# matthewhoung/inference-arena

Measured on AMD Instinct MI355X. Metric: req/sec (whole node) + P50/P99 e2e latency, YOLOv5n→MobileNetV2 at 1/2/4/8 GPU, higher is better.
Workload: dtype fp32

## Files before the change

### csrc/kernels/conv_f32.hip

```cpp
#include <algorithm>
#include <cstdlib>
#include <stdexcept>
#include <string>

#include "common.h"
#include "launch.h"
#include "letterbox.h"

namespace arena {

__device__ __forceinline__ float4 load_f4_or_zero(const float* p, const float* safe, bool ok) {
  const float4 v = *(const float4*)(ok ? p : safe);
  return ok ? v : make_float4(0.f, 0.f, 0.f, 0.f);
}

__device__ __forceinline__ float f4_get(const float4& v, int s) {
  return s == 0 ? v.x : s == 1 ? v.y : s == 2 ? v.z : v.w;
}

__device__ __forceinline__ int xcd_remap(int bx, int nx) {
  const int q = nx / 8, r = nx % 8, x = bx % 8, y = bx / 8;
  return (x < r ? x * (q + 1) : r * (q + 1) + (x - r) * q) + y;
}

// ... 1351 lines not shown
}

static bool f32_stream(const ConvParams& p, hipStream_t s) {
  if (p.Cin % 4 != 0 || p.Kpad > 192 || p.Kpad % 16 != 0 || p.Kpad < p.KH * p.KW * p.Cin || p.xs % 4 != 0)
    return false;
  const int ncf = p.Cout_pad / 16;
  const int nf = ncf <= 5 ? ncf : ncf % 4 == 0 ? 4 : ncf % 3 == 0 ? 3 : ncf % 5 == 0 ? 5 : ncf % 2 == 0 ? 2 : 1;
  switch (nf) {
    case 1: return launch_stream_exact_k<1>(p, s);
    case 2: return launch_stream_exact_k<2>(p, s);
    case 3: return launch_stream_exact_k<3>(p, s);
    case 4: return launch_stream_exact_k<4>(p, s);
    case 5: return launch_stream_exact_k<5>(p, s);
    default: return false;
  }
}

static bool x3_stream(const ConvParams& p, hipStream_t s, int nf_force) {
  if (p.Cin % 8 != 0 || p.Kpad > 192 || p.Kpad < p.KH * p.KW * p.Cin || p.xs % 4 != 0) return false;
  const int ncf = p.Cout_pad / 16;
  const int nf = nf_force ? nf_force
                          : ncf <= 5 ? ncf : ncf % 4 == 0 ? 4 : ncf % 3 == 0 ? 3 : ncf % 5 == 0 ? 5 : ncf % 2 == 0 ? 2 : 1;
  switch (nf) {
    case 1: return launch_stream_k<1>(p, s);
    case 2: return launch_stream_k<2>(p, s);
    case 3: return launch_stream_k<3>(p, s);
    case 4: return launch_stream_k<4>(p, s);
    case 5: return launch_stream_k<5>(p, s);
    default: return false;
  }
}

void conv2d_f32(const ConvParams& p, hipStream_t s) {
  if (p.Cin % 4 != 0 || p.xs % 4 != 0 || p.Kpad % 16 != 0 || p.Cout_pad % 16 != 0 || p.Cout % 4 != 0 ||
      p.Cout > p.Cout_pad || p.ys % 4 != 0)
    throw std::runtime_error("conv2d_f32: unsupported geometry (Cin/xs/ys %4, Kpad %16, Cout_pad %16, Cout %4)");
  if (p.Cin < 16) throw std::runtime_error("conv2d_f32: Cin must be >= 16");
  if (p.Kpad < p.KH * p.KW * p.Cin) throw std::runtime_error("conv2d_f32: Kpad < KH*KW*Cin");
  if (p.pw_w != nullptr) {
    if (p.impl >= kF32X3HRPw && p.impl < kF32X3HRPw + kF32X3HRPwVariants) {
      if (!conv_x3hr_pw(p, s, p.impl - kF32X3HRPw))
        throw std::runtime_error("conv2d_f32: a fused pointwise epilogue needs an x3hr-pw variant that fits the conv");
      return;
    }
    const int v = p.impl >= kF32X3HGPw && p.impl < kF32X3HGPw + kF32X3HGPwVariants ? p.impl - kF32X3HGPw
                  : p.impl >= kF32X3HGPwSmall && p.impl < kF32X3HGPwSmall + kF32X3HGPwSmallVariants
                      ? kF32X3HGPwVariants + p.impl - kF32X3HGPwSmall
                  : p.impl == 0 ? (p.Cout_pad <= 64 ? 0 : 2)
                                : -1;
    if (v < 0 || !conv_x3hg_pw(p, s, v))
      throw std::runtime_error("conv2d_f32: a fused pointwise epilogue needs an x3hg-pw variant that fits the conv");
    return;
  }
  if (p.res != nullptr && p.rs % 4 != 0) throw std::runtime_error("conv2d_f32: residual stride % 4");
  if (p.y2 != nullptr && p.y2s % 4 != 0) throw std::runtime_error("conv2d_f32: upsampled stride % 4");
  const long M = (long)p.B * p.Ho * p.Wo;
  if (M <= 0) return;
  if (M > 0x7fffffffL || (long)p.B * p.H * p.W * p.xs > 0x7fffffffL) throw std::runtime_error("conv2d_f32: too large");
  const int ncf = p.Cout_pad / 16;
  if (p.lb_meta != nullptr) {
    if (p.lb_pool == nullptr || !x3_h16(p, s))
      throw std::runtime_error("conv2d_f32: a letterbox-source conv must be a 3x3 s1 pad-1 conv over 16 channels");
    return;
  }
  if (p.impl >= 10) {
    if (p.impl >= kF32X3G && p.impl < kF32X3G + kF32X3GVariants) {
      if (!conv_x3g(p, s, p.impl - kF32X3G))
        throw std::runtime_error("conv2d_f32: not an x3g-eligible conv (needs pre-split weights)");
      return;
    }
    if (p.impl >= kF32X3GSK && p.impl < kF32X3GSK + kF32X3GSKVariants) {
      if (!conv_x3g_sk(p, s, p.impl - kF32X3GSK))
        throw std::runtime_error("conv2d_f32: not a split-K x3g-eligible conv (pre-split weights, workspace)");
      return;
    }
    if (p.impl >= kF32X3HG && p.impl < kF32X3HG + kF32X3HGVariants) {
      if (!conv_x3hg(p, s, p.impl - kF32X3HG))
        throw std::runtime_error("conv2d_f32: not an x3hg-eligible conv (3x3 s1 with pre-split weights)");
      return;
    }
    if (p.impl >= kF32X3HR && p.impl < kF32X3HR + kF32X3HRVariants) {
      if (!conv_x3hr(p, s, p.impl - kF32X3HR))
        throw std::runtime_error("conv2d_f32: not an x3hr-eligible conv (3x3 s1 with pre-split weights)");
      return;
    }
    if (p.impl == kF32X3H16) {
      if (!x3_h16(p, s)) throw std::runtime_error("conv2d_f32: not an x3-h16-eligible conv (3x3 s1 over 16 channels)");
      return;
    }
    if (p.impl == kF32Fc) {
      if (!conv_fc_f32(p, s)) throw std::runtime_error("conv2d_f32: not an FC-eligible conv (1x1 map, Kpad 1280)");
      return;
    }
    if (p.impl == kF32StreamExact) {
      if (!f32_stream(p, s)) throw std::runtime_error("conv2d_f32: not a stream-eligible conv (Cin % 4, Kpad <= 192)");
      return;
    }
    if (p.impl == kF32Stream || p.impl == kF32StreamN2) {
      if (!x3_stream(p, s, p.impl == kF32StreamN2 ? 2 : 0))
        throw std::runtime_error("conv2d_f32: not a stream-eligible conv (Cin % 8, Kpad <= 192)");
      return;
    }
    if (p.impl == kF32X3Halo || p.impl == kF32X3HaloN3 || p.impl == kF32X3HaloN2 || p.impl == kF32X3Halo16 ||
        p.impl == kF32X3Halo16N3) {
      const int nf = (p.impl == kF32X3HaloN3 || p.impl == kF32X3Halo16N3) ? 3 : p.impl == kF32X3HaloN2 ? 2 : 0;
      const int th = (p.impl == kF32X3Halo16 || p.impl == kF32X3Halo16N3) ? 16 : 8;
      if (!x3_halo(p, s, nf, th)) throw std::runtime_error("conv2d_f32: not an x3-halo-eligible conv");
      return;
    }
    if (p.impl == kF32Halo) {
      if (!halo_f32(p, s, true)) throw std::runtime_error("conv2d_f32: not a halo-eligible conv");
      return;
    }
    if (p.impl >= kF32X3) {
      if (p.impl >= kF32X3 + kF32X3Variants || !launch_x3_variant(p, s, M, p.impl - kF32X3))
        throw std::runtime_error("conv2d_f32: unknown x3 variant");
      return;
    }
    if (p.impl >= 10 + kF32Variants || !launch_lds_variant(p, s, M, p.impl - 10)) throw std::runtime_error("conv2d_f32: unknown variant");
    return;
  }
  if (p.impl == 0 && conv_fc_f32(p, s)) return;
  const int impl = p.impl == 1 ? 1 : p.impl >= 2 ? 2 : f32_conv_family();
  if (impl == 2 && halo_f32(p, s)) return;
  if (impl == 2) {
    if (ncf == 1)
      launch_lds_m<1, 4, 1>(p, s, M);
    else if (ncf == 2)
      launch_lds_m<2, 4, 1>(p, s, M);
    else if (ncf == 3 || ncf == 9)
      launch_lds_m<3, 4, 1>(p, s, M);
    else if (ncf == 5)
      launch_lds_m<5, 4, 1>(p, s, M);
    else if (ncf == 6)
      launch_lds_m<3, 2, 2>(p, s, M);
    else
      launch_lds_m<2, 2, 2>(p, s, M);
    return;
  }
  if (ncf % 4 == 0 || ncf > 12)
    launch_f32_wc<4>(p, s, M);
  else if (ncf % 3 == 0)
    launch_f32_wc<3>(p, s, M);
  else if (ncf % 2 == 0)
    launch_f32_wc<2>(p, s, M);
  else if (ncf == 5)
    launch_f32_wc<5>(p, s, M);
  else
    launch_f32_wc<1>(p, s, M);
}

template <int R, int S, int CX>
__global__ __launch_bounds__(256) void dwconv_f32_kernel(const DwParams p) {
  const int B = live_batch(p.B, p.bdev);
  const int cg = p.C >> 2;
  const int strips = (p.Ho + R - 1) / R;
  const int colb = (p.Wo + CX - 1) / CX;
  const int total = B * strips * colb * cg;
  const int tid = blockIdx.x * blockDim.x + threadIdx.x;
  if (tid >= total) return;
  const int g = tid % cg;
  int t = tid / cg;
  const int ox0 = (t % colb) * CX;
  t /= colb;
  const int st = t % strips;
  const int b = t / strips;
// ... 151 lines not shown
```

### csrc/kernels/detect.hip

```cpp
#include <string>
#include <stdexcept>
#include "common.h"
#include "launch.h"

namespace arena {

constexpr int SPPF_MAX_PIX = 1024;

__global__ __launch_bounds__(256) void sppf_kernel(const SppfParams p) {
  extern __shared__ __align__(16) uint4 sp[];
  const int B = live_batch(p.B, p.bdev);
  const int groups = p.C >> 4;
  const int b = blockIdx.x / groups;
  if (b >= B) return;
  const int c0 = (blockIdx.x - b * groups) * 16;
  const int H = p.H, W = p.W, HW = H * W;
  uint4* in = sp;
  uint4* h5 = sp + 2 * HW;
  uint4* h9 = sp + 4 * HW;
  uint4* h13 = sp + 6 * HW;
  bf16* buf = (bf16*)p.buf + (size_t)b * HW * p.xs;
  constexpr int kIt = (SPPF_MAX_PIX * 2 + 255) / 256;
  uint4 tmp[kIt];
#pragma unroll
// ... 171 lines not shown
  int P = 2;
  while (P < n) P <<= 1;
  unsigned long long* keys = (unsigned long long*)smem;
  unsigned char* removed = smem + sizeof(unsigned long long) * P;
  const Candidate* cand = p.cand + (size_t)b * p.cand_cap;

  for (int i = tid; i < P; i += NMS_THREADS) {
    unsigned long long k = ~0ull;
    if (i < n) {
      const Candidate c = cand[i];
      const unsigned bits = __float_as_uint(c.score);
      unsigned diff = bits <= 0x3F800000u ? 0x3F800000u - bits : 0u;
      diff = diff < (1u << 29) ? diff : (1u << 29) - 1u;
      k = ((unsigned long long)(unsigned)(c.cls & 127) << 57) | ((unsigned long long)diff << 28) |
          ((unsigned long long)(unsigned)(c.anchor & 0x3FFF) << 14) | (unsigned long long)i;
      removed[i] = 0;
    }
    keys[i] = k;
  }
  __syncthreads();
  for (int k = 2; k <= P; k <<= 1) {
    for (int j = k >> 1; j > 0; j >>= 1) {
      for (int i = tid; i < P; i += NMS_THREADS) {
        const int ixj = i ^ j;
        if (ixj > i) {
          const unsigned long long a = keys[i], c = keys[ixj];
          const bool up = (i & k) == 0;
          if ((a > c) == up) { keys[i] = c; keys[ixj] = a; }
        }
      }
      __syncthreads();
    }
  }

  const ImageMeta m = p.meta[b];
  const float scale = m.scale;
  int kept = 0;
  for (int i = 0; i < n; ++i) {
    if (removed[i]) continue;
    const unsigned long long ki = keys[i];
    const int ci = (int)(ki >> 57);
    const Candidate bi = cand[ki & 0x3FFF];
    if (tid == 0 && kept < p.max_det) {
      Detection d;
      d.x1 = fminf(fmaxf((bi.x1 - (float)m.pad_w) / scale, 0.f), (float)m.w);
      d.y1 = fminf(fmaxf((bi.y1 - (float)m.pad_h) / scale, 0.f), (float)m.h);
      d.x2 = fminf(fmaxf((bi.x2 - (float)m.pad_w) / scale, 0.f), (float)m.w);
      d.y2 = fminf(fmaxf((bi.y2 - (float)m.pad_h) / scale, 0.f), (float)m.h);
      d.conf = bi.score;
      d.cls = bi.cls;
      d.pad_[0] = d.pad_[1] = 0.f;
      p.det[(size_t)b * p.max_det + kept] = d;
    }
    ++kept;
    const float area_i = (bi.x2 - bi.x1) * (bi.y2 - bi.y1);
    for (int j = i + 1 + tid; j < n; j += NMS_THREADS) {
      const unsigned long long kj = keys[j];
      if ((int)(kj >> 57) != ci) break;
      if (removed[j]) continue;
      const Candidate bj = cand[kj & 0x3FFF];
      const float xx1 = fmaxf(bi.x1, bj.x1), yy1 = fmaxf(bi.y1, bj.y1);
      const float xx2 = fminf(bi.x2, bj.x2), yy2 = fminf(bi.y2, bj.y2);
      const float inter = fmaxf(0.f, xx2 - xx1) * fmaxf(0.f, yy2 - yy1);
      const float area_j = (bj.x2 - bj.x1) * (bj.y2 - bj.y1);
      const float iou = inter / (area_i + area_j - inter + 1e-6f);
      if (iou > p.iou_thr) removed[j] = 1;
    }
    __syncthreads();
  }
  if (tid == 0) p.det_count[b] = kept;
}

void prepare_kernels() {
  static bool done = false;
  if (done) return;
  ARENA_HIP_CHECK(hipFuncSetAttribute((const void*)nms_kernel, hipFuncAttributeMaxDynamicSharedMemorySize,
                                      160 * 1024));
  ir_prepare();
  head_pool_f32_prepare();
  x3_halo_prepare();
  x3g_prepare();
  c3_x3_prepare();
  x3hg_prepare();
  stem_s2_f32_prepare();
  ARENA_HIP_CHECK(hipFuncSetAttribute((const void*)sppf_kernel, hipFuncAttributeMaxDynamicSharedMemorySize,
                                      160 * 1024));
  done = true;
}

void nms(const NmsParams& p, hipStream_t s) {
  if (p.cand_cap > 16384) throw std::runtime_error("nms: cand_cap > 16384");
  int P = 2;
  while (P < p.cand_cap) P <<= 1;
  const size_t lds = (size_t)P * 9;
  if (lds > 160 * 1024) throw std::runtime_error("nms: LDS budget exceeded");
  if (p.B <= 0) return;
  hipLaunchKernelGGL(nms_kernel, dim3(p.B), dim3(NMS_THREADS), lds, s, p);
}

__global__ __launch_bounds__(256) void crop_plan_kernel(const CropPlanParams p) {
  __shared__ int offs[1024 + 1];
  const int n_img = live_batch(p.B, p.ctrl ? &p.ctrl->n_images : nullptr);
  const int tid = threadIdx.x;
  if (p.whole) {
    for (int b = tid; b < n_img; b += blockDim.x) {
      const ImageMeta m = p.meta[b];
      Detection d;
      d.x1 = 0.f; d.y1 = 0.f; d.x2 = (float)m.w; d.y2 = (float)m.h;
      d.conf = 1.f; d.cls = -1; d.pad_[0] = d.pad_[1] = 0.f;
      p.det[(size_t)b * p.max_det] = d;
      p.det_count[b] = 1;
      CropRef r;
      r.img = b; r.x1 = 0; r.y1 = 0; r.x2 = m.w; r.y2 = m.h; r.det = 0; r.pad_[0] = r.pad_[1] = 0;
      p.crops[b] = r;
    }
    if (tid == 0) {
      Ctrl* c = p.ctrl;
      c->total_crops = n_img;
      int rem = n_img - c->crop_base;
      rem = rem < 0 ? 0 : rem;
      c->n_crops = rem < p.crop_cap ? rem : p.crop_cap;
    }
    return;
  }
  for (int b = tid; b < n_img; b += blockDim.x) {
    const int k = p.det_count[b];
    offs[b + 1] = k < p.max_det ? k : p.max_det;
  }
  if (tid == 0) offs[0] = 0;
  __syncthreads();
  if (tid < 64) {
    int carry = 0;
    for (int base = 0; base < n_img; base += 64) {
      const int i = base + tid;
      int v = i < n_img ? offs[i + 1] : 0;
#pragma unroll
      for (int o = 1; o < 64; o <<= 1) {
        const int u = __shfl_up(v, o, 64);
        if (tid >= o) v += u;
      }
      if (i < n_img) offs[i + 1] = v + carry;
      carry += __shfl(v, 63, 64);
    }
    if (tid == 0) {
      Ctrl* c = p.ctrl;
      c->total_crops = carry;
      int rem = carry - c->crop_base;
      rem = rem < 0 ? 0 : rem;
      c->n_crops = rem < p.crop_cap ? rem : p.crop_cap;
    }
  }
  __syncthreads();
  const int total = offs[n_img];
  for (int i = tid; i < total; i += blockDim.x) {
    int lo = 0, hi = n_img - 1;
    while (lo < hi) {
      const int mid = (lo + hi + 1) >> 1;
      if (offs[mid] <= i) lo = mid;
      else hi = mid - 1;
    }
    const int b = lo, d = i - offs[lo];
    const ImageMeta m = p.meta[b];
    const Detection det = p.det[(size_t)b * p.max_det + d];
    CropRef r;
    r.img = b;
    r.x1 = max(0, (int)det.x1);
// ... 78 lines not shown
```

### csrc/kernels/launch.h

```cpp
#pragma once
#include <hip/hip_runtime.h>
#include <stdint.h>
#include <stdexcept>
#include <string>

namespace arena {

struct ImageMeta;
struct CropRef;
struct Ctrl;
struct ConvParams {
  const void* x;
  int B, H, W;
  int xs;
  int Cin;
  const void* w;
  int Kpad;
  const float* bias;
  void* y;
  int Ho, Wo, ys;
  int Cout;
  int Cout_pad;
  int KH, KW, stride, pad_t, pad_l;
  const void* res;
  int rs;
  void* y2;
  int y2s;
  int act;
  int f32out;
  const int* bdev;
  int impl;
  const void* pw_w;
  const float* pw_bias;
  void* pw_y;
  int pw_ys, pw_cout, pw_kpad, pw_act;
  const uint8_t* lb_pool;
  const ImageMeta* lb_meta;
  const void* w3;
  float* sk_ws;
  int64_t sk_ws_bytes;
  int sk_splits;
};
void conv2d(const ConvParams& p, hipStream_t s);
void conv_igemm(const ConvParams& p, hipStream_t s);
bool conv_pw(const ConvParams& p, hipStream_t s);
void set_conv_pw(bool v);
bool conv3x3_v3(const ConvParams& p, hipStream_t s);
bool conv_fc(const ConvParams& p, hipStream_t s);
void set_conv_v3(bool v);
void set_conv_impl(int v);
int get_conv_impl();

constexpr int kF32Variants = 16;
constexpr int kF32X3 = 40;
constexpr int kF32X3Variants = 12;
constexpr int kF32Halo = 100;
constexpr int kF32X3Halo = 101;
constexpr int kF32X3HaloN3 = 102;
constexpr int kF32X3HaloN2 = 103;
constexpr int kF32Stream = 104;
constexpr int kF32StreamN2 = 105;
constexpr int kF32Fc = 106;
constexpr int kF32StreamExact = 107;
constexpr int kF32X3Halo16 = 108;
constexpr int kF32X3Halo16N3 = 109;
constexpr int kF32X3H16 = 110;
constexpr int kF32X3G = 111;
constexpr int kF32X3GVariants = 20;
void x3_halo_prepare();
bool x3g_supported(const ConvParams& p);
bool conv_x3g(const ConvParams& p, hipStream_t s, int v);
constexpr int kF32X3GSK = 171;
constexpr int kF32X3GSKVariants = 9;
bool conv_x3g_sk(const ConvParams& p, hipStream_t s, int v);
void x3g_prepare();
constexpr int kF32X3HG = 131;
constexpr int kF32X3HGVariants = 14;
bool x3hg_supported(const ConvParams& p);
bool conv_x3hg(const ConvParams& p, hipStream_t s, int v);
void x3hg_prepare();
constexpr int kF32X3HGPw = 145;
constexpr int kF32X3HGPwVariants = 6;
constexpr int kF32X3HGPwSmall = 181;
constexpr int kF32X3HGPwSmallVariants = 2;
bool conv_x3hg_pw(const ConvParams& p, hipStream_t s, int v);
constexpr int kF32X3HR = 151;
constexpr int kF32X3HRVariants = 10;
constexpr int kF32X3HRPw = 161;
constexpr int kF32X3HRPwVariants = 6;
bool conv_x3hr(const ConvParams& p, hipStream_t s, int v);
bool conv_x3hr_pw(const ConvParams& p, hipStream_t s, int v);
bool conv_fc_f32(const ConvParams& p, hipStream_t s);
void conv2d_f32(const ConvParams& p, hipStream_t s);

struct DwParams {
  const void* x;
  int B, H, W, xs, C;
  const void* w;
  const float* bias;
  void* y;
  int Ho, Wo, ys, stride, act;
  const int* bdev;
};
void dwconv3x3(const DwParams& p, hipStream_t s);
void dwconv3x3_f32(const DwParams& p, hipStream_t s);

struct IrParams {
  const void* x;
  int x_cs, H, W;
  int inp, inp_pad;
  int hid_pad;
  int oup, oup_pad;
  int stride, expand, res;
  const void* we;
  const float* be;
  const void* wd;
  const float* bd;
  const void* wp;
  const float* bp;
  void* y;
  int y_cs, Ho, Wo;
  int B;
  const int* bdev;
  int x3w;
  int x_parts, y_parts;
  int stem;
  const uint8_t* st_pool;
  const ImageMeta* st_meta;
  const CropRef* st_crops;
  const Ctrl* st_ctrl;
  int st_S;
  float st_mean[3], st_inv_std[3];
  const float* st_w;
  const float* st_b;
};
void ir_block(const IrParams& p, hipStream_t s);
void ir_block_f32(const IrParams& p, hipStream_t s);
bool ir_block_f32_supported(int stride, int inp_pad, int hid_pad, int oup_pad, int expand);
bool ir_block_crop_f32(const IrParams& p, hipStream_t s);
bool ir_block_crop_f32_supported(int H, int stride, int inp_pad, int hid_pad, int oup_pad, int expand);
bool ir_tile_x3(const IrParams& p, hipStream_t s);
bool ir_tile_x3_supported(int stride, int inp_pad, int hid_pad, int oup_pad, int expand);
void ir_tile_x3_prepare();
bool ir_stem_x3(const IrParams& p, hipStream_t s);
void ir_prepare();
void set_ir_t14(bool v);
void set_ir_crop(bool v);
void set_ir_crop_split(int v);
void set_ir_wave(bool v);
void set_irx_slices_big(int n);
void set_irx_parts(int n);

struct C3Params {
  const void* x;
  int xs;
  int B, H, W;
  const int* bdev;
  int C1, CH, NB, res;
  const void* w12;
  const float* b12;
  const void* wb1[2];
  const float* bb1[2];
  const void* wb2[2];
  const float* bb2[2];
  const void* w3;
  const float* b3;
  void* y;
  int ys;
};
bool c3_fused_supported(int C1, int CH, int NB, bool res, int H, int W);
bool c3_x3_supported(int C1, int CH, int NB, bool res, int H, int W);
void c3_x3(const C3Params& p, hipStream_t s);
// ... 221 lines not shown
```

### csrc/runtime/executor.cpp

```cpp
#include "executor.h"
#include "peer.h"

#include <pthread.h>
#include <sys/prctl.h>

#include <algorithm>
#include <chrono>
#include <cmath>
#include <cstdio>
#include <cstdlib>
#include <cstring>
#include <thread>
#include <stdexcept>
#include <string>

#include "../kernels/common.h"
#include "../kernels/jpeg_desc.h"
#include "jpeg_decode.h"
#include "trace.h"

namespace arena {

namespace {
float bits_to_float(int64_t v) {
// ... 219 lines not shown

std::vector<uint8_t> Executor::weights_host() {
  std::vector<uint8_t> out(weights_bytes_);
  if (d_weights_ == nullptr || weights_bytes_ == 0) return out;
  ARENA_HIP_CHECK(hipSetDevice(cfg_.device));
  sync_slots();
  ARENA_HIP_CHECK(hipMemcpy(out.data(), d_weights_, weights_bytes_, hipMemcpyDeviceToHost));
  return out;
}

void Executor::set_program(const int64_t* ops, int n_ops, const int64_t* cls_ops, int n_cls_ops) {
  prog_.resize(n_ops);
  for (int i = 0; i < n_ops; ++i) std::memcpy(prog_[i].data(), ops + (size_t)i * kOpFields, sizeof(OpRecord));
  cls_prog_.resize(n_cls_ops);
  for (int i = 0; i < n_cls_ops; ++i)
    std::memcpy(cls_prog_[i].data(), cls_ops + (size_t)i * kOpFields, sizeof(OpRecord));
  has_topk_ = has_det_ = has_raw_ = has_stamps_ = false;
  for (const auto& r : prog_) {
    has_topk_ |= r[0] == OP_TOPK;
    has_stamps_ |= r[0] == OP_STAMP;
    has_det_ |= r[0] == OP_NMS || r[0] == OP_CROPPLAN;
    for (int f = 1; f < kOpFields; ++f) has_raw_ |= r[f] == BUF_RAWOUT && (r[0] == OP_YOLORAW || r[0] == OP_CONV);
  }
  if (has_raw_ && cfg_.raw_out_bytes <= 0) throw std::runtime_error("program exports raw outputs: raw_out_bytes = 0");
}

int Executor::crop_cap_for(int B) const { return std::max(cfg_.min_crop_cap, B * cfg_.crop_cap_per_image); }

std::vector<int> Executor::buckets() const {
  std::vector<int> r;
  for (auto& kv : buckets_) r.push_back(kv.first);
  return r;
}

uintptr_t Executor::arena_ptr(int B) const {
  auto it = buckets_.find(B);
  return it == buckets_.end() ? 0 : (uintptr_t)it->second.d_arena[0];
}

void Executor::read_arena(int B, int64_t offset, void* dst, size_t bytes) {
  auto it = buckets_.find(B);
  if (it == buckets_.end()) throw std::runtime_error("read_arena: unknown bucket");
  if (offset < 0 || offset + (int64_t)bytes > it->second.info.arena_bytes)
    throw std::runtime_error("read_arena: range outside the arena");
  ARENA_HIP_CHECK(hipSetDevice(cfg_.device));
  sync_slots();
  ARENA_HIP_CHECK(hipMemcpy(dst, it->second.d_arena[it->second.last_slot] + offset, bytes, hipMemcpyDeviceToHost));
}

void Executor::add_bucket(int B, const int64_t* offsets, int n_buffers, int64_t arena_bytes,
                          const std::vector<int>* impl) {
  if (B <= 0 || B > max_B_) throw std::runtime_error("add_bucket: B outside (0, max_batch]");
  if (prog_.empty()) throw std::runtime_error("add_bucket: set_program first");
  if (d_weights_ == nullptr) throw std::runtime_error("add_bucket: set_weights first");
  ARENA_HIP_CHECK(hipSetDevice(cfg_.device));
  Bucket& bk = buckets_[B];
  bk.info.B = B;
  bk.info.crop_cap = crop_cap_for(B);
  bk.info.offsets.assign(offsets, offsets + n_buffers);
  bk.info.arena_bytes = arena_bytes;
  sync_slots();
  free_arenas(bk);
  const size_t abytes = (size_t)std::max<int64_t>(arena_bytes, 256);
  for (int s = 0; s < n_slots_; ++s) {
    ARENA_HIP_CHECK(hipMalloc(&bk.d_arena[s], abytes));
    ARENA_HIP_CHECK(hipMemset(bk.d_arena[s], 0, abytes));
  }
  bk.impl.assign(prog_.size(), 0);
  if (impl != nullptr) {
    if (impl->size() != prog_.size()) throw std::runtime_error("add_bucket: tuning table does not match the program");
    for (size_t i = 0; i < prog_.size(); ++i) {
      const int v = (*impl)[i];
      const bool f32 = prog_[i][kDtypeField] == 1;
      const bool ok = f32 ? (v >= 0 && v <= 2) || (v >= 10 && v < 10 + kF32Variants) ||
                                (v >= kF32X3 && v < kF32X3 + kF32X3Variants) || v == kF32Halo || v == kF32X3Halo ||
                                v == kF32X3HaloN3 || v == kF32X3HaloN2 || v == kF32Stream || v == kF32StreamN2 ||
                                v == kF32Fc || v == kF32StreamExact || v == kF32X3Halo16 || v == kF32X3Halo16N3 ||
                                v == kF32X3H16 || (v >= kF32X3G && v < kF32X3G + kF32X3GVariants) ||
                                (v >= kF32X3HG && v < kF32X3HG + kF32X3HGVariants) ||
                                (v >= kF32X3HGPw && v < kF32X3HGPw + kF32X3HGPwVariants) ||
                                (v >= kF32X3HGPwSmall && v < kF32X3HGPwSmall + kF32X3HGPwSmallVariants) ||
                                (v >= kF32X3HR && v < kF32X3HR + kF32X3HRVariants) ||
                                (v >= kF32X3HRPw && v < kF32X3HRPw + kF32X3HRPwVariants) ||
                                (v >= kF32X3GSK && v < kF32X3GSK + kF32X3GSKVariants)
                          : v >= 0 && v <= 3;
      if (!ok || (v != 0 && prog_[i][0] != OP_CONV)) throw std::runtime_error("add_bucket: bad tuning entry");
      bk.impl[i] = (int16_t)v;
    }
  } else if (autotune_) {
    autotune(bk);
  }
  for (int s = 0; s < n_slots_; ++s) capture(bk, s);
  if (debug_sync_ || std::getenv("ARENA_DEBUG_ALLOC")) {
    fprintf(stderr, "[arena alloc] bucket %d arena %p..%p (%lld B)\n", B, (void*)bk.d_arena[0],
            (void*)(bk.d_arena[0] + arena_bytes), (long long)arena_bytes);
    for (int s = 0; s < n_slots_; ++s)
      fprintf(stderr, "[arena alloc] slot %d in %p..%p out %p..%p\n", s, (void*)slots_[s].d_in,
              (void*)(slots_[s].d_in + in_bytes_total()), (void*)slots_[s].d_out,
              (void*)(slots_[s].d_out + out_bytes_total()));
    fprintf(stderr, "[arena alloc] weights %p..%p\n", (void*)d_weights_, (void*)(d_weights_ + weights_bytes_));
  }
}

void Executor::autotune(Bucket& bk) {
  Slot& sl = slots_[0];
  Ctrl c{};
  c.n_images = bk.info.B;
  c.n_crops = bk.info.crop_cap;
  ARENA_HIP_CHECK(hipStreamSynchronize(compute_));
  ARENA_HIP_CHECK(hipMemcpy(sl.d_in, &c, sizeof(Ctrl), hipMemcpyHostToDevice));
  hipEvent_t e0, e1;
  ARENA_HIP_CHECK(hipEventCreate(&e0));
  ARENA_HIP_CHECK(hipEventCreate(&e1));
  static const int kF32Candidates[] = {0,      12,     13,     14,     17,     19,     20,         21,
                                       23,     24,     kF32Halo, kF32X3, kF32X3 + 1, kF32X3 + 4, kF32X3 + 5,
                                       kF32X3 + 6, kF32X3 + 7, kF32X3 + 8, kF32X3Halo, kF32X3HaloN3,
                                       kF32X3HaloN2, kF32Stream, kF32StreamN2, kF32Fc, kF32StreamExact,
                                       kF32X3Halo16, kF32X3Halo16N3, kF32X3H16,
                                       kF32X3G + 5, kF32X3G + 6, kF32X3G + 7, kF32X3G + 9, kF32X3G + 15,
                                       kF32X3G + 16, kF32X3G + 17, kF32X3G + 19,
                                       kF32X3HG + 0, kF32X3HG + 1, kF32X3HG + 2, kF32X3HG + 4, kF32X3HG + 6,
                                       kF32X3HG + 7, kF32X3HG + 8, kF32X3HG + 9, kF32X3HG + 10,
                                       kF32X3HGPw + 0, kF32X3HGPw + 1, kF32X3HGPw + 2, kF32X3HGPw + 3,
                                       kF32X3HGPw + 4, kF32X3HGPw + 5, kF32X3HGPwSmall + 0, kF32X3HGPwSmall + 1,
                                       kF32X3HR + 0, kF32X3HR + 1, kF32X3HR + 2, kF32X3HR + 3, kF32X3HR + 4,
                                       kF32X3HR + 5, kF32X3HR + 6, kF32X3HR + 7, kF32X3HR + 8, kF32X3HR + 9,
                                       kF32X3HRPw + 0, kF32X3HRPw + 1, kF32X3HRPw + 2, kF32X3HRPw + 3,
                                       kF32X3HRPw + 4, kF32X3HRPw + 5,
                                       kF32X3GSK + 0, kF32X3GSK + 1, kF32X3GSK + 2, kF32X3GSK + 3, kF32X3GSK + 4,
                                       kF32X3GSK + 5, kF32X3GSK + 6, kF32X3GSK + 7, kF32X3GSK + 8};
  static const int kBf16Candidates[] = {1, 2, 3};
  for (size_t i = 0; i < prog_.size(); ++i) {
    if (prog_[i][0] != OP_CONV) continue;
    const bool f32 = prog_[i][kDtypeField] == 1;
    if (prog_[i][1] == BUF_POOL) {
      bk.impl[i] = kF32X3H16;
      continue;
    }
    if (!f32 && prog_[i][34] > 0) {
      bk.impl[i] = 2;
      continue;
    }
    const int reps = f32 ? 5 : 3;
    std::vector<OpRecord> one(1, prog_[i]);
    float best = 1e30f;
    int best_impl = -1;
    const int* cand = f32 ? kF32Candidates : kBf16Candidates;
    const int n_cand = f32 ? (int)(sizeof(kF32Candidates) / sizeof(int)) : 3;
    for (int ci = 0; ci < n_cand; ++ci) {
      const int impl = cand[ci];
      try {
        enqueue_program(one, bk, sl, compute_, (int)i, impl);
      } catch (const std::runtime_error&) {
        continue;
      }
      ARENA_HIP_CHECK(hipEventRecord(e0, compute_));
      for (int k = 0; k < reps; ++k) enqueue_program(one, bk, sl, compute_, (int)i, impl);
      ARENA_HIP_CHECK(hipEventRecord(e1, compute_));
      ARENA_HIP_CHECK(hipEventSynchronize(e1));
      float ms = 0.f;
      ARENA_HIP_CHECK(hipEventElapsedTime(&ms, e0, e1));
      if (best_impl < 0 || ms < best * 0.97f) {
        best = ms;
        best_impl = impl;
      }
    }
    bk.impl[i] = (int16_t)std::max(best_impl, 0);
    if (autotune_ > 1)
      fprintf(stderr, "[arena autotune] B=%d op %zu -> impl %d (%.1f us)\n", bk.info.B, i, best_impl,
              best * 1e3f / reps);
  }
  ARENA_HIP_CHECK(hipEventDestroy(e0));
  ARENA_HIP_CHECK(hipEventDestroy(e1));
  ARENA_HIP_CHECK(hipMemset(bk.d_arena[0], 0, std::max<int64_t>(bk.info.arena_bytes, 256)));
}

static int lanes_max_batch() {
  static const int v = [] {
    const char* e = std::getenv("ARENA_LANES_MAX_BATCH");
    return e != nullptr ? std::atoi(e) : 2;
  }();
  return v;
}

bool Executor::lanes_for(const Bucket& bk) const {
  if (bk.info.B > lanes_max_batch()) return false;
  for (const OpRecord& r : prog_)
    if (r[kLaneField] >= 1 && r[kLaneField] <= kMaxLanes) return true;
  return false;
}

int64_t Executor::sk_lane_bytes() {
  static const int64_t v = [] {
    const char* e = std::getenv("ARENA_SPLITK_WS_MB");
    return (int64_t)std::max(1, e != nullptr ? std::atoi(e) : 16) << 20;
  }();
  return v;
}

void Executor::destroy_graphs(Bucket& bk, int s) {
  if (bk.graph[s]) hipGraphExecDestroy(bk.graph[s]);
  bk.graph[s] = nullptr;
  for (hipGraphExec_t g : bk.parts[s])
    if (g) hipGraphExecDestroy(g);
  bk.parts[s].clear();
  for (auto& sg : bk.segs[s])
    if (sg.g) hipGraphExecDestroy(sg.g);
  bk.segs[s].clear();
}

void Executor::capture(Bucket& bk, int s) {
// ... 1094 lines not shown
```

Before: 10310.

## Add register-prefetched halo 3x3 conv kernel family to fp32 autotune candidates

Adds a new 3x3 stride-1 fp32 conv kernel (x3hp) that stages an input halo tile and weight slices in LDS as bf16x3 splits and uses six MFMA products to emulate fp32 accuracy. Global loads for the next stage are issued into registers before the MFMA work of the current stage, so memory latency can overlap compute. Nine tile and stage variants are registered with the dispatcher and added to the autotune candidate list. The effect depends on the autotuner choosing these variants over existing ones; it adds compile time and LDS pressure per variant.

```diff
diff --git a/csrc/kernels/conv_f32.hip b/csrc/kernels/conv_f32.hip
--- a/csrc/kernels/conv_f32.hip
+++ b/csrc/kernels/conv_f32.hip
@@ -1457,6 +1457,11 @@
     if (p.impl >= kF32X3HR && p.impl < kF32X3HR + kF32X3HRVariants) {
       if (!conv_x3hr(p, s, p.impl - kF32X3HR))
         throw std::runtime_error("conv2d_f32: not an x3hr-eligible conv (3x3 s1 with pre-split weights)");
+      return;
+    }
+    if (p.impl >= kF32X3HP && p.impl < kF32X3HP + kF32X3HPVariants) {
+      if (!conv_x3hp(p, s, p.impl - kF32X3HP))
+        throw std::runtime_error("conv2d_f32: not an x3hp-eligible conv (3x3 s1 with pre-split weights)");
       return;
     }
     if (p.impl == kF32X3H16) {
diff --git a/csrc/kernels/detect.hip b/csrc/kernels/detect.hip
--- a/csrc/kernels/detect.hip
+++ b/csrc/kernels/detect.hip
@@ -277,6 +277,7 @@
   x3g_prepare();
   c3_x3_prepare();
   x3hg_prepare();
+  x3hp_prepare();
   stem_s2_f32_prepare();
   ARENA_HIP_CHECK(hipFuncSetAttribute((const void*)sppf_kernel, hipFuncAttributeMaxDynamicSharedMemorySize,
                                       160 * 1024));
diff --git a/csrc/kernels/halo_x3p.hip b/csrc/kernels/halo_x3p.hip
--- /dev/null
+++ b/csrc/kernels/halo_x3p.hip
@@ -0,0 +1,259 @@
+#include <stdexcept>
+#include <string>
+
+#include "common.h"
+#include "launch.h"
+
+namespace arena {
+
+namespace {
+
+typedef unsigned u32x4 __attribute__((ext_vector_type(4)));
+
+constexpr int HP_TW = 16, HP_HC = HP_TW + 2;
+constexpr int HP_XP = 3 * 32 + 16;
+__host__ __device__ constexpr int hp_wp(int TS) { return TS * 96 + 16; }
+__host__ __device__ constexpr int hp_lds_bytes(int NF, int TH, int TS) {
+  return ((TH + 2) * HP_HC * HP_XP + NF * 16 * hp_wp(TS)) * 2;
+}
+
+__device__ __forceinline__ int hp_xcd_remap(int bx, int nx) {
+  const int q = nx / 8, r = nx % 8, x = bx % 8, y = bx / 8;
+  return (x < r ? x * (q + 1) : r * (q + 1) + (x - r) * q) + y;
+}
+
+}
+
+template <int NF, int TH, int TS>
+__global__ __launch_bounds__(TH * 32) void conv_x3hp_kernel(const ConvParams p) {
+  static_assert(TS == 1 || TS == 3, "a weight stage is one tap or one kernel row");
+  constexpr int NT = TH * 32, NW = TH / 2;
+  constexpr int HR = TH + 2, HPIX = HR * HP_HC;
+  constexpr int XI = (HPIX * 8 + NT - 1) / NT;
+  constexpr int BN = NF * 16, MF = 2;
+  constexpr int WP = hp_wp(TS);
+  constexpr int WPC = TS * BN * 12;
+  constexpr int WI = (WPC + NT - 1) / NT;
+  constexpr int SPC = 9 / TS;
+  extern __shared__ __attribute__((aligned(16))) bf16 hp_lds[];
+  bf16* sX = hp_lds;
+  bf16* sW = hp_lds + HPIX * HP_XP;
+
+  const int tid = threadIdx.x, lane = tid & 63, wave = tid >> 6;
+  const int col = lane & 15, kq = lane >> 4;
+  const int tiles_x = (p.Wo + HP_TW - 1) / HP_TW, tiles_y = (p.Ho + TH - 1) / TH;
+  const int tiles = tiles_x * tiles_y;
+  const int bx = hp_xcd_remap(blockIdx.x, gridDim.x);
+  const int b = bx / tiles;
+  if (b >= live_batch(p.B, p.bdev)) return;
+  const int t = bx - b * tiles;
+  const int ty = t / tiles_x, tx = t - ty * tiles_x;
+  const int oy0 = ty * TH, ox0 = tx * HP_TW;
+  const int iy0 = oy0 - p.pad_t, ix0 = ox0 - p.pad_l;
+  const int n0 = blockIdx.y * BN;
+  const int H = p.H, W = p.W, Cin = p.Cin;
+
+  const __amdgpu_buffer_rsrc_t xr = __builtin_amdgcn_make_buffer_rsrc(
+      const_cast<void*>(p.x), (short)0, (int)((size_t)p.B * H * W * p.xs * 4), 0x00020000);
+  const int cin32 = (Cin + 31) >> 5;
+  const __amdgpu_buffer_rsrc_t wr = __builtin_amdgcn_make_buffer_rsrc(
+      const_cast<void*>(p.w3), (short)0, (int)((size_t)9 * cin32 * p.Cout_pad * 192), 0x00020000);
+  constexpr int kOob = 0x7fffffff & ~15;
+
+  int x_off[XI];
+  const size_t img = (size_t)b * H * W;
+#pragma unroll
+  for (int j = 0; j < XI; ++j) {
+    const int i = tid + NT * j;
+    const int px = i >> 3, g = i & 7;
+    const int hy = px / HP_HC, hx = px - hy * HP_HC;
+    const int iy = iy0 + hy, ix = ix0 + hx;
+    const bool in = i < HPIX * 8 && (unsigned)iy < (unsigned)H && (unsigned)ix < (unsigned)W;
+    x_off[j] = in ? (int)(((img + (size_t)iy * W + ix) * p.xs + 4 * g) * 4) : kOob;
+  }
+  int w_off[WI], w_dst[WI];
+  const int tap_bytes = cin32 * p.Cout_pad * 192;
+#pragma unroll
+  for (int j = 0; j < WI; ++j) {
+    const int i = tid + NT * j;
+    const int kxl = i / (BN * 12), r = i - kxl * (BN * 12);
+    const int row = r / 12, piece = r - row * 12;
+    const int n = n0 + row;
+    w_off[j] = (i < WPC && n < p.Cout_pad) ? kxl * tap_bytes + n * 192 + piece * 16 : kOob;
+    w_dst[j] = row * WP + kxl * 96 + piece * 8;
+  }
+
+  f32x4 rx[XI];
+  u32x4 rw[WI];
+  auto load_x = [&](int c0) {
+#pragma unroll
+    for (int j = 0; j < XI; ++j) {
+      const int c = c0 + 4 * ((tid + NT * j) & 7);
+      const int o = (x_off[j] != kOob && c < Cin) ? x_off[j] + 4 * c0 : kOob;
+      rx[j] = __builtin_bit_cast(f32x4, __builtin_amdgcn_raw_buffer_load_b128(xr, o, 0, 0));
+    }
+  };
+  auto store_x = [&]() {
+#pragma unroll
+    for (int j = 0; j < XI; ++j) {
+      const int i = tid + NT * j;
+      if (HPIX * 8 % NT == 0 || i < HPIX * 8) {
+        bf16x2 h0, m0, l0, h1, m1, l1;
+        split_bf16x3_pair(f32x2{rx[j][0], rx[j][1]}, h0, m0, l0);
+        split_bf16x3_pair(f32x2{rx[j][2], rx[j][3]}, h1, m1, l1);
+        bf16* d = sX + (i >> 3) * HP_XP + 4 * (i & 7);
+        *(bf16x4*)d = __builtin_shufflevector(h0, h1, 0, 1, 2, 3);
+        *(bf16x4*)(d + 32) = __builtin_shufflevector(m0, m1, 0, 1, 2, 3);
+        *(bf16x4*)(d + 64) = __builtin_shufflevector(l0, l1, 0, 1, 2, 3);
+      }
+    }
+  };
+  auto load_w = [&](int st) {
+    const int chunk = st / SPC, s = st - chunk * SPC;
+    const int step = (s * TS * cin32 + chunk) * p.Cout_pad * 192;
+#pragma unroll
+    for (int j = 0; j < WI; ++j) rw[j] = __builtin_amdgcn_raw_buffer_load_b128(wr, w_off[j], step, 0);
+  };
+  auto store_w = [&]() {
+#pragma unroll
+    for (int j = 0; j < WI; ++j)
+      if (WPC % NT == 0 || tid + NT * j < WPC) *(u32x4*)(sW + w_dst[j]) = rw[j];
+  };
+
+  f32x4 acc[MF][NF];
+#pragma unroll
+  for (int f = 0; f < MF; ++f)
+#pragma unroll
+    for (int j = 0; j < NF; ++j) acc[f][j] = f32x4{0.f, 0.f, 0.f, 0.f};
+
+  const int nstage = cin32 * SPC;
+  load_x(0);
+  load_w(0);
+  for (int st = 0; st < nstage; ++st) {
+    const int chunk = st / SPC, s = st - chunk * SPC;
+    if (s == 0) store_x();
+    store_w();
+    __syncthreads();
+    if (st + 1 < nstage) {
+      if (s == SPC - 1) load_x((chunk + 1) * 32);
+      load_w(st + 1);
+    }
+    const int ky = TS == 3 ? s : s / 3;
+#pragma unroll
+    for (int kxl = 0; kxl < TS; ++kxl) {
+      const int kx = TS == 3 ? kxl : s - ky * 3;
+      bf16x8 bh[MF], bm[MF], bl[MF];
+#pragma unroll
+      for (int f = 0; f < MF; ++f) {
+        const int oy = wave + NW * f;
+        const bf16* r = &sX[((oy + ky) * HP_HC + col + kx) * HP_XP + 8 * kq];
+        bh[f] = *(const bf16x8*)r;
+        bm[f] = *(const bf16x8*)(r + 32);
+        bl[f] = *(const bf16x8*)(r + 64);
+      }
+#pragma unroll
+      for (int j = 0; j < NF; ++j) {
+        const bf16* r = &sW[(j * 16 + col) * WP + kxl * 96 + 8 * kq];
+        const bf16x8 ah = *(const bf16x8*)r;
+        const bf16x8 am = *(const bf16x8*)(r + 32);
+        const bf16x8 al = *(const bf16x8*)(r + 64);
+#pragma unroll
+        for (int f = 0; f < MF; ++f) {
+          f32x4 c = acc[f][j];
+          c = __builtin_amdgcn_mfma_f32_16x16x32_bf16(am, bm[f], c, 0, 0, 0);
+          c = __builtin_amdgcn_mfma_f32_16x16x32_bf16(al, bh[f], c, 0, 0, 0);
+          c = __builtin_amdgcn_mfma_f32_16x16x32_bf16(ah, bl[f], c, 0, 0, 0);
+          c = __builtin_amdgcn_mfma_f32_16x16x32_bf16(am, bh[f], c, 0, 0, 0);
+          c = __builtin_amdgcn_mfma_f32_16x16x32_bf16(ah, bm[f], c, 0, 0, 0);
+          acc[f][j] = __builtin_amdgcn_mfma_f32_16x16x32_bf16(ah, bh[f], c, 0, 0, 0);
+        }
+      }
+    }
+    __syncthreads();
+  }
+
+  const int HWo = p.Ho * p.Wo;
+#pragma unroll
+  for (int j = 0; j < NF; ++j) {
+    const int cb = n0 + j * 16 + kq * 4;
+    if (cb >= p.Cout) continue;
+    const float4 bias = *(const float4*)(p.bias + cb);
+#pragma unroll
+    for (int f = 0; f < MF; ++f) {
+      const int oy = oy0 + wave + NW * f, ox = ox0 + col;
+      if (oy >= p.Ho || ox >= p.Wo) continue;
+      const size_t pix = (size_t)b * HWo + (size_t)oy * p.Wo + ox;
+      float v[4] = {acc[f][j][0] + bias.x, acc[f][j][1] + bias.y, acc[f][j][2] + bias.z, acc[f][j][3] + bias.w};
+#pragma unroll
+      for (int r = 0; r < 4; ++r) v[r] = apply_act(v[r], p.act);
+      if (p.res != nullptr) {
+        const float4 rv = *(const float4*)((const float*)p.res + pix * p.rs + cb);
+        v[0] += rv.x; v[1] += rv.y; v[2] += rv.z; v[3] += rv.w;
+      }
+      const float4 o = make_float4(v[0], v[1], v[2], v[3]);
+      *(float4*)((float*)p.y + pix * p.ys + cb) = o;
+      if (p.y2 != nullptr) {
+        const int W2 = 2 * p.Wo;
+        float* y2 = (float*)p.y2;
+        const size_t base = ((size_t)(b * 2 * p.Ho + 2 * oy) * W2 + 2 * ox);
+        *(float4*)(y2 + base * p.y2s + cb) = o;
+        *(float4*)(y2 + (base + 1) * p.y2s + cb) = o;
+        *(float4*)(y2 + (base + W2) * p.y2s + cb) = o;
+        *(float4*)(y2 + (base + W2 + 1) * p.y2s + cb) = o;
+      }
+    }
+  }
+}
+
+namespace {
+
+template <int NF, int TH, int TS>
+void hp_launch(const ConvParams& p, hipStream_t s) {
+  constexpr int BN = NF * 16;
+  const int tiles = ((p.Wo + HP_TW - 1) / HP_TW) * ((p.Ho + TH - 1) / TH);
+  dim3 grid((unsigned)(p.B * tiles), (unsigned)((p.Cout_pad + BN - 1) / BN));
+  hipLaunchKernelGGL((conv_x3hp_kernel<NF, TH, TS>), grid, dim3(TH * 32), hp_lds_bytes(NF, TH, TS), s, p);
+}
+
+#define HP_VARIANTS(X) \
+  X(0, 2, 8, 3)    \
+  X(1, 3, 8, 3)    \
+  X(2, 4, 8, 3)    \
+  X(3, 5, 8, 3)    \
+  X(4, 2, 16, 3)   \
+  X(5, 3, 16, 3)   \
+  X(6, 4, 16, 3)   \
+  X(7, 9, 8, 1)    \
+  X(8, 9, 16, 1)
+
+}
+
+bool x3hp_supported(const ConvParams& p) {
+  const size_t x_bytes = (size_t)p.B * p.H * p.W * p.xs * 4;
+  const size_t w_bytes = (size_t)9 * ((p.Cin + 31) / 32) * p.Cout_pad * 192;
+  return p.w3 != nullptr && p.KH == 3 && p.KW == 3 && p.stride == 1 && p.Cin % 4 == 0 && p.xs % 4 == 0 &&
+         x_bytes < (1u << 31) - (1u << 20) && w_bytes < (1u << 31) - (1u << 20) && p.Cout % 4 == 0 &&
+         p.Cout_pad % 16 == 0 && p.ys % 4 == 0 && (p.res == nullptr || p.rs % 4 == 0) &&
+         (p.y2 == nullptr || p.y2s % 4 == 0) && p.lb_meta == nullptr && p.pw_w == nullptr;
+}
+
+bool conv_x3hp(const ConvParams& p, hipStream_t s, int v) {
+  if (!x3hp_supported(p)) return false;
+  switch (v) {
+#define HP_CASE(V, NF, TH, TS) \
+  case V: hp_launch<NF, TH, TS>(p, s); return true;
+    HP_VARIANTS(HP_CASE)
+#undef HP_CASE
+    default: return false;
+  }
+}
+
+void x3hp_prepare() {
+#define HP_ATTR(V, NF, TH, TS)                                                                      \
+  ARENA_HIP_CHECK(hipFuncSetAttribute((const void*)conv_x3hp_kernel<NF, TH, TS>,                     \
+                                      hipFuncAttributeMaxDynamicSharedMemorySize, hp_lds_bytes(NF, TH, TS)));
+  HP_VARIANTS(HP_ATTR)
+#undef HP_ATTR
+}
+
+}
diff --git a/csrc/kernels/launch.h b/csrc/kernels/launch.h
--- a/csrc/kernels/launch.h
+++ b/csrc/kernels/launch.h
@@ -88,6 +88,11 @@
 constexpr int kF32X3HRVariants = 10;
 constexpr int kF32X3HRPw = 161;
 constexpr int kF32X3HRPwVariants = 6;
+constexpr int kF32X3HP = 191;
+constexpr int kF32X3HPVariants = 9;
+bool x3hp_supported(const ConvParams& p);
+bool conv_x3hp(const ConvParams& p, hipStream_t s, int v);
+void x3hp_prepare();
 bool conv_x3hr(const ConvParams& p, hipStream_t s, int v);
 bool conv_x3hr_pw(const ConvParams& p, hipStream_t s, int v);
 bool conv_fc_f32(const ConvParams& p, hipStream_t s);
diff --git a/csrc/runtime/executor.cpp b/csrc/runtime/executor.cpp
--- a/csrc/runtime/executor.cpp
+++ b/csrc/runtime/executor.cpp
@@ -325,6 +325,7 @@
                                 (v >= kF32X3HGPwSmall && v < kF32X3HGPwSmall + kF32X3HGPwSmallVariants) ||
                                 (v >= kF32X3HR && v < kF32X3HR + kF32X3HRVariants) ||
                                 (v >= kF32X3HRPw && v < kF32X3HRPw + kF32X3HRPwVariants) ||
+                                (v >= kF32X3HP && v < kF32X3HP + kF32X3HPVariants) ||
                                 (v >= kF32X3GSK && v < kF32X3GSK + kF32X3GSKVariants)
                           : v >= 0 && v <= 3;
       if (!ok || (v != 0 && prog_[i][0] != OP_CONV)) throw std::runtime_error("add_bucket: bad tuning entry");
@@ -370,6 +371,8 @@
                                        kF32X3HR + 5, kF32X3HR + 6, kF32X3HR + 7, kF32X3HR + 8, kF32X3HR + 9,
                                        kF32X3HRPw + 0, kF32X3HRPw + 1, kF32X3HRPw + 2, kF32X3HRPw + 3,
                                        kF32X3HRPw + 4, kF32X3HRPw + 5,
+                                       kF32X3HP + 0, kF32X3HP + 1, kF32X3HP + 2, kF32X3HP + 3, kF32X3HP + 4,
+                                       kF32X3HP + 5, kF32X3HP + 6, kF32X3HP + 7, kF32X3HP + 8,
                                        kF32X3GSK + 0, kF32X3GSK + 1, kF32X3GSK + 2, kF32X3GSK + 3, kF32X3GSK + 4,
                                        kF32X3GSK + 5, kF32X3GSK + 6, kF32X3GSK + 7, kF32X3GSK + 8};
   static const int kBf16Candidates[] = {1, 2, 3};
```

Result: faster. 10500 (median of 6 runs) (+1.8%).
